# AnnaLew/pangenomix

Measured on AMD Instinct MI355X. Metric: proteins/sec clustered at 0.8 identity + pan/core iters/sec, 400-genome set, higher is better.
Workload: dtype i32

## Files before the change

pangenomix_amd/csrc/cluster.hip:

```cpp
#include <algorithm>
#include <chrono>
#include <cstdlib>
#include <cmath>
#include <type_traits>
#include <functional>
#include <condition_variable>
#include <mutex>
#include <thread>
#include <vector>

#include "cluster_layout.h"
#include "cluster_tables.h"
#include "pgx_internal.h"

namespace {

using namespace pgxc;

constexpr uint32_t kWindowMax = 65536;
constexpr int kDiscoveryRounds = 2;
constexpr uint32_t kBlockCap = 4096;
constexpr uint32_t kBlockCapMin = 64;

constexpr uint32_t kMaxLen = 1u << 22;
// ... 20 lines not shown
    uint32_t minc;
    int32_t best_sum, band_left, band_center, band_right;
    int32_t iden;
    uint32_t flags;
};

struct PairSel {
    const uint32_t *d_begin, *d_end;
    uint32_t cap;
    const uint32_t *list;
    uint32_t n_list;
    const uint8_t *only_a, *only_not_b;
    uint8_t *accepted_out;
    uint32_t b0;
    uint32_t skip_evaluated;
    uint32_t all_if_le;
};
__device__ __forceinline__ uint32_t sel_count(const PairSel &s) {
    if (s.list) return s.n_list;
    uint32_t e = *s.d_end;
    if (e > s.cap) e = s.cap;
    const uint32_t b = s.d_begin ? *s.d_begin : 0u;
    return e > b ? e - b : 0u;
}
__device__ __forceinline__ uint32_t sel_pair(const PairSel &s, uint32_t w) {
    return s.list ? s.list[w] : (s.d_begin ? *s.d_begin : 0u) + w;
}

struct DevSeqs {
    const uint8_t *res;
    const uint64_t *off;
    const uint32_t *len;
    const uint32_t *wcode;
    const uint16_t *wmult;
    const uint32_t *wcnt;
    const uint32_t *pk;
    const uint32_t *pk_off;
    uint32_t n_fwd;
    int32_t base;
    int32_t kd;
    int32_t nt;
    uint32_t mshift;
};
__device__ __forceinline__ uint32_t entry_rmask(const DevSeqs &S) { return (1u << S.mshift) - 1u; }
__device__ __forceinline__ uint32_t entry_fmax(const DevSeqs &S) { return 0xFFFFFFFFu >> S.mshift; }
__device__ __forceinline__ uint32_t real_of(const DevSeqs &S, uint32_t k) { return k >= S.n_fwd ? k - S.n_fwd : k; }

__constant__ int8_t kAa2Idx_dev[26] = {0, 2, 4, 3, 6, 13, 7, 8, 9, 20, 11, 10, 12,
                                       2, 20, 14, 5, 1, 15, 16, 20, 19, 17, 20, 18, 6};

__device__ __forceinline__ bool is_letter(uint8_t ch) {
    ch &= 0xDF;
    return ch >= 'A' && ch <= 'Z';
}

__global__ __launch_bounds__(256) void seq_len_kernel(const uint8_t *__restrict__ res,
                                                     const uint64_t *__restrict__ off, uint32_t n, uint64_t total,
                                                     uint32_t *__restrict__ len) {
    const uint32_t lane = threadIdx.x & 63u;
    const uint32_t i = blockIdx.x * 4u + (threadIdx.x >> 6);
    if (i >= n) return;
    const uint64_t b = off[i], e = off[i + 1];
    uint32_t c = 0;
    const uint64_t a0 = b & ~3ull;
    for (uint64_t a = a0 + 4ull * lane; a < e; a += 256) {
        uint32_t word = 0;
        if (a + 4 <= total) word = *reinterpret_cast<const uint32_t *>(res + a);
        else for (uint64_t p = a; p < total; ++p) word |= (uint32_t)res[p] << (8 * (p - a));
#pragma unroll
        for (int t = 0; t < 4; ++t) {
            const uint64_t p = a + t;
            c += (p >= b && p < e) && is_letter((uint8_t)(word >> (8 * t)));
        }
    }
    for (int d = 32; d > 0; d >>= 1) c += __shfl_xor(c, d);
    if (lane == 0) len[i] = c;
}

__global__ __launch_bounds__(256) void encode_gather_kernel(const uint8_t *__restrict__ in,
                                                           const uint64_t *__restrict__ in_off,
                                                           const uint32_t *__restrict__ order,
                                                           const uint64_t *__restrict__ out_off,
                                                           uint8_t *__restrict__ out, uint32_t n, int nt) {
    const uint32_t lane = threadIdx.x & 63u;
    const uint32_t k = blockIdx.x * 4u + (threadIdx.x >> 6);
    if (k >= n) return;
    const uint32_t src = order[k];
    const uint64_t b = in_off[src], e = in_off[src + 1];
    uint64_t w = out_off[k];
    for (uint64_t q0 = b; q0 < e; q0 += 256) {
        uint8_t chs[4];
#pragma unroll
        for (int j = 0; j < 4; ++j) { const uint64_t p = q0 + 64u * j + lane; chs[j] = p < e ? in[p] : (uint8_t)0; }
#pragma unroll
        for (int j = 0; j < 4; ++j) {
            const uint8_t ch = chs[j];
            const bool ok = is_letter(ch);
            const unsigned long long m = __ballot(ok);
            if (ok) {
                const uint8_t up = ch & 0xDF;
                const uint8_t idx = nt ? (uint8_t)(up == 'A' ? 0 : up == 'C' ? 1 : up == 'G' ? 2 : (up == 'T' || up == 'U') ? 3 : 4)
                                       : (uint8_t)kAa2Idx_dev[up - 'A'];
                out[w + __popcll(m & ((1ull << lane) - 1ull))] = idx;
            }
            w += __popcll(m);
        }
// ... 279 lines not shown
            if (cur == key) break;
            if (cur == kSentinel) {
                const uint32_t was = atomicCAS(&hk[slot], kSentinel, key);
                if (was == kSentinel || was == key) break;
            }
            slot = (slot + 1u) & (SLOTS - 1u);
        }
        atomicAdd(&hc[slot], 1u);
    }
    __syncthreads();
    constexpr uint32_t C = SLOTS / THREADS;
    const uint32_t beg = tid * C;
    uint32_t mine = 0;
    for (uint32_t i = beg; i < beg + C; ++i) mine += hk[i] != kSentinel;
    uint32_t total;
    uint32_t idx = block_excl_scan<THREADS>(mine, part, &total);
    if (tid == 0) wcnt[k] = total;
    for (uint32_t i = beg; i < beg + C; ++i)
        if (hk[i] != kSentinel) { wcode[o + idx] = hk[i]; wmult[o + idx] = (uint16_t)hc[i]; ++idx; }
}

template <uint32_t SLOTS>
__global__ __launch_bounds__(256) void words_wave_kernel(const uint8_t *__restrict__ res, const uint64_t *__restrict__ off,
                                                         const uint32_t *__restrict__ len, uint32_t k0, uint32_t k1,
                                                         int word_len, int base, int nt, uint32_t *__restrict__ wcode,
                                                         uint16_t *__restrict__ wmult, uint32_t *__restrict__ wcnt) {
    constexpr uint32_t kStage = (15 + SLOTS / 2 + 10 + 15) / 16 + 1;
    constexpr uint32_t kLoads = (kStage + 63) / 64;
    __shared__ uint4 table4[4][SLOTS / 4];
    __shared__ uint4 stage[4][kStage];
    const uint32_t lane = threadIdx.x & 63u, wv = threadIdx.x >> 6;
    const uint32_t k = k0 + blockIdx.x * 4u + wv;
    if (k >= k1) return;
    const uint64_t o = off[k];
    const uint32_t L = len[k], nw = L - (uint32_t)word_len + 1u;
    const uint8_t *s = res + o;
    const uint8_t *g = reinterpret_cast<const uint8_t *>(reinterpret_cast<uintptr_t>(s) & ~uintptr_t(15));
    const uint32_t sh = (uint32_t)(s - g), nv = (sh + L + 15u) / 16u;
    uint4 v[kLoads];
#pragma unroll
    for (uint32_t t = 0; t < kLoads; ++t) {
        v[t] = make_uint4(0, 0, 0, 0);
        if (lane + 64u * t < nv && lane + 64u * t < kStage) v[t] = reinterpret_cast<const uint4 *>(g)[lane + 64u * t];
    }
    uint32_t *tb = reinterpret_cast<uint32_t *>(table4[wv]);
#pragma unroll
    for (uint32_t t = 0; t < SLOTS / 4 / 64; ++t) table4[wv][lane + 64u * t] = make_uint4(kSentinel, kSentinel, kSentinel, kSentinel);
#pragma unroll
    for (uint32_t t = 0; t < kLoads; ++t) if (lane + 64u * t < kStage) stage[wv][lane + 64u * t] = v[t];
    __builtin_amdgcn_fence(__ATOMIC_RELEASE, "workgroup");
    __builtin_amdgcn_wave_barrier();
    __builtin_amdgcn_fence(__ATOMIC_ACQUIRE, "workgroup");
    const uint8_t *l = reinterpret_cast<const uint8_t *>(stage[wv]) + sh;
    for (uint32_t i = lane; i < nw; i += 64u) {
        uint32_t key = 0;
        bool bad = false;
        for (int t = 0; t < word_len; ++t) { const uint32_t r = l[i + t]; key = key * (uint32_t)base + r; bad |= r >= (uint32_t)base; }
        if (nt && bad) continue;
        uint32_t slot = (key * 0x9E3779B1u) >> 7 & (SLOTS - 1u);
        for (;;) {
            const uint32_t cur = tb[slot];
            if (cur != kSentinel && (cur >> 10) == key) { atomicAdd(&tb[slot], 1u); break; }
            if (cur == kSentinel) {
                const uint32_t was = atomicCAS(&tb[slot], kSentinel, key << 10 | 1u);
                if (was == kSentinel) break;
                if ((was >> 10) == key) { atomicAdd(&tb[slot], 1u); break; }
            }
            slot = (slot + 1u) & (SLOTS - 1u);
        }
    }
    __builtin_amdgcn_fence(__ATOMIC_RELEASE, "workgroup");
    __builtin_amdgcn_wave_barrier();
    __builtin_amdgcn_fence(__ATOMIC_ACQUIRE, "workgroup");
    uint32_t n_out = 0;
#pragma unroll 4
    for (uint32_t r = 0; r < SLOTS / 64u; ++r) {
        const uint32_t e = tb[r * 64u + lane];
        const bool occ = e != kSentinel;
        const unsigned long long m = __ballot(occ);
        if (occ) {
            const uint32_t at = n_out + (uint32_t)__popcll(m & ((1ull << lane) - 1ull));
            wcode[o + at] = e >> 10;
            wmult[o + at] = (uint16_t)(e & 1023u);
        }
        n_out += (uint32_t)__popcll(m);
    }
    if (lane == 0) wcnt[k] = n_out;
}

__global__ __launch_bounds__(1024) void words_huge_kernel(const uint8_t *__restrict__ res, const uint64_t *__restrict__ off,
                                                          const uint32_t *__restrict__ len, uint32_t k0, uint32_t k1,
                                                          int word_len, int base, int nt, uint32_t *__restrict__ scratch,
                                                          uint32_t slots, uint32_t *__restrict__ wcode,
                                                          uint16_t *__restrict__ wmult, uint32_t *__restrict__ wcnt,
                                                          uint32_t *__restrict__ err) {
    __shared__ uint32_t part[1024];
    const uint32_t k = k0 + blockIdx.x;
    if (k >= k1) return;
    const uint32_t tid = threadIdx.x;
    uint32_t *hk = scratch + (size_t)blockIdx.x * 2u * slots, *hc = hk + slots;
    const uint64_t o = off[k];
    const uint8_t *s = res + o;
    const uint32_t nw = len[k] - (uint32_t)word_len + 1u;
    for (uint32_t i = tid; i < slots; i += 1024) { hk[i] = kSentinel; hc[i] = 0u; }
    __threadfence();
    __syncthreads();
// ... 1618 lines not shown
        return 1e3 * std::chrono::duration<double>(std::chrono::steady_clock::now() - t).count();
    };
    const bool trace_phases = std::getenv("PGX_TRACE") != nullptr;
    double t_mark = 0.0;
    auto phase = [&](const char *what) {
        if (!trace_phases) return;
        const double now = ms_since(t_call0);
        fprintf(stderr, "[pgx] %-28s %8.2f ms\n", what, now - t_mark);
        t_mark = now;
    };
    pgx_cluster_stats S{};
    S.n_input = n_in;
    if (out_n_clusters) *out_n_clusters = 0;
    const unsigned nth = host_threads(n_in);
    parallel_for(n_in, nth, [&](unsigned, size_t b, size_t e) {
        for (size_t i = b; i < e; ++i) {
            out_cluster[i] = -1; out_member[i] = -1; out_identity[i] = 0.f;
            if (out_strand) out_strand[i] = 0;
        }
    });
    if (n_in == 0) { if (stats) *stats = S; return PGX_OK; }

    DevBuf d_res, d_off, d_len, d_wcode, d_wmult, d_wcnt, d_aa1, d_aas, d_aan, d_lines, d_pool[2], d_idx,
        d_newbits, d_touched, d_first, d_best_own, d_rcvis, d_counters, d_visits, d_pairsW, d_pairsK, d_blk_list,
        d_ulist, d_new_list, d_flags, d_gscratch, d_order, d_list, d_gather, d_pk, d_pkoff,
        d_counters2, d_best2, d_flags2, d_pairsW2, d_gscratch2,
        d_thr, d_hugewords, d_xsend, d_xrecv,
        d_hist, d_sortcnt, d_tilesum, d_runs;
    {
        DevBuf *all[] = {&d_res, &d_off, &d_len, &d_wcode, &d_wmult, &d_wcnt, &d_aa1, &d_aas, &d_aan, &d_lines,
                         &d_pool[0], &d_pool[1], &d_idx, &d_newbits, &d_touched, &d_first, &d_best_own, &d_rcvis,
                         &d_counters, &d_visits, &d_pairsW, &d_pairsK, &d_blk_list, &d_ulist, &d_new_list, &d_flags,
                         &d_gscratch, &d_order, &d_list, &d_gather, &d_pk, &d_pkoff,
                         &d_counters2, &d_best2, &d_flags2, &d_pairsW2, &d_gscratch2, &d_thr, &d_hugewords,
                         &d_xsend, &d_xrecv, &d_hist, &d_sortcnt, &d_tilesum, &d_runs};
        int sl = 1;
        for (DevBuf *b : all) { b->ctx = ctx; b->slot = sl++; }
    }
    uint32_t n_codes = 1;
    for (int t = 0; t < P->word_len; ++t) n_codes *= nt ? 4u : (uint32_t)kNAA1;
    static_assert(kSegs == 4, "eight codes per word of the round's map");
    const uint32_t bm_words = (n_codes / 8 + 2 + 3) & ~3u;
    const bool overlap = !nt && !std::getenv("PGX_NO_OVERLAP");
    DevBuf d_in_len;
    d_in_len.ctx = ctx; d_in_len.slot = 0;
    PGX_HIP(d_in_len.alloc((size_t)n_in * 4));
    constexpr uint32_t kHistWords = H_BINS + kDevSortMaxLen + 1;
    PGX_HIP(d_hist.alloc((size_t)kHistWords * 4));
    PGX_HIP(d_idx.alloc(16));
    PGX_HIP(d_newbits.alloc(2 * (size_t)bm_words * 4 + 16));
    PGX_HIP(d_counters.alloc(C_COUNT * 4));
    PGX_HIP(d_visits.alloc(8));
    if (overlap) PGX_HIP(d_counters2.alloc(C_COUNT * 4));
    {
        ClearArgs ca{};
        auto seg = [&](DevBuf &b, size_t words) { ca.p[ca.n] = b.as<uint32_t>(); ca.words[ca.n] = (uint32_t)words; ++ca.n; };
        seg(d_hist, kHistWords);
        seg(d_newbits, 2 * (size_t)bm_words);
        seg(d_counters, C_COUNT);
        seg(d_visits, 2);
        if (overlap) seg(d_counters2, C_COUNT);
        ca.one = d_idx.as<uint32_t>();
        clear_kernel<<<1024, 256, 0, st>>>(ca);
        LAUNCH_CHECK();
    }
    {
        ProfScope prof(ctx, "seq_len_kernel", st);
        seq_len_kernel<<<(n_in + 3) / 4, 256, 0, st>>>(d_residues, d_offsets, n_in, total_in, d_in_len.as<uint32_t>());
        len_hist_kernel<<<std::min(64u, (n_in + 1023u) / 1024u), 1024, 0, st>>>(d_in_len.as<uint32_t>(), n_in, P->min_length,
                                                                               d_hist.as<uint32_t>());
    }
    LAUNCH_CHECK();
    HostVec<uint32_t> h_hist(ctx, 6, kHistWords);
    PGX_REQUIRE(h_hist.ok(), "out of host memory");
    PGX_HIP(hipMemcpyAsync(h_hist.data(), d_hist.p, (size_t)(H_BINS + kHistLds) * 4, hipMemcpyDeviceToHost, st));
    PGX_HIP(hipStreamSynchronize(st));
    const bool dev_sort = h_hist[H_OVER] == 0 && !std::getenv("PGX_HOST_PROLOGUE");
    uint32_t max_len = h_hist[H_MAX];
    if (dev_sort && max_len >= kHistLds) {
        PGX_HIP(hipMemcpyAsync(h_hist.data() + H_BINS + kHistLds, d_hist.as<uint32_t>() + H_BINS + kHistLds,
                               (size_t)(max_len + 1 - kHistLds) * 4, hipMemcpyDeviceToHost, st));
        PGX_HIP(hipStreamSynchronize(st));
    }
    phase("  seq_len + histogram + copy");
    const uint32_t *len_hist = h_hist.data() + H_BINS;
    uint32_t n = 0;
    HostVec<uint32_t> order(ctx, 1, dev_sort ? 0 : n_in);
    std::vector<uint32_t> host_hist;
    if (dev_sort) {
        for (uint32_t L = 0; L <= max_len; ++L) n += len_hist[L];
    } else {
        HostVec<uint32_t> in_len(ctx, 0, n_in);
        PGX_REQUIRE(in_len.ok() && order.ok(), "out of host memory");
        PGX_HIP(hipMemcpyAsync(in_len.data(), d_in_len.p, (size_t)n_in * 4, hipMemcpyDeviceToHost, st));
        PGX_HIP(hipStreamSynchronize(st));
        max_len = 0;
        {
            std::vector<uint32_t> mx(nth, 0u);
            parallel_for(n_in, nth, [&](unsigned t, size_t b, size_t e) {
                uint32_t m = 0;
                for (size_t i = b; i < e; ++i) m = std::max(m, in_len[i]);
                mx[t] = m;
            });
            for (uint32_t m : mx) max_len = std::max(max_len, m);
        }
        if (max_len > kMaxLen) {
            pgx_set_error("pgx_cluster_greedy: sequence of %u residues exceeds the supported maximum %u", max_len, kMaxLen);
            return PGX_ERR_CAPACITY;
        }
        const size_t n_bkt = (size_t)max_len + 2;
        std::vector<uint32_t> bucket(n_bkt * nth, 0);
        parallel_for(n_in, nth, [&](unsigned t, size_t b, size_t e) {
            uint32_t *h = bucket.data() + n_bkt * t;
            for (size_t i = b; i < e; ++i)
                if ((int)in_len[i] > P->min_length) h[max_len - in_len[i]]++;
        });
        host_hist.assign((size_t)max_len + 1, 0u);
        for (size_t l = 0; l <= max_len; ++l)
            for (unsigned t = 0; t < nth; ++t) {
                const uint32_t c = bucket[n_bkt * t + l];
                bucket[n_bkt * t + l] = n; n += c; host_hist[max_len - l] += c;
            }
        parallel_for(n_in, nth, [&](unsigned t, size_t b, size_t e) {
            uint32_t *h = bucket.data() + n_bkt * t;
            for (size_t i = b; i < e; ++i)
                if ((int)in_len[i] > P->min_length) order[h[max_len - in_len[i]]++] = (uint32_t)i;
        });
        len_hist = host_hist.data();
    }
// ... 45 lines not shown
            PGX_REQUIRE(!(len_hist[L] && t_aas[L] < 1), "aas_cutoff too small: every sequence needs required_aas >= 1");
        S.sum_len_queries = run_off[n_runs];
    }
    S.n_clustered = n;

    const uint32_t window_cap = pgx_cluster_window_cap(P);
    PGX_REQUIRE(!exchanging || window_cap <= PGX_EXCHANGE_KEYS, "window larger than PGX_EXCHANGE_KEYS");
    uint32_t pair_cap = 4u << 20;
    uint32_t block_cap = std::min(nt ? 512u : kBlockCap, window_cap);
    const uint32_t pair_cap_k = nt ? 512u * 512u + 16u : (1u << 20);
    const double thr_frac = P->identity > 0.95 ? std::max(0.0, 1.0 - (1.0 - P->identity) * P->word_len) : P->aan_cutoff;
    static const double chunk_frac = std::getenv("PGX_CHUNK_FRAC") ? std::atof(std::getenv("PGX_CHUNK_FRAC")) : 0.8;
    double cur_frac = chunk_frac;
    uint64_t chunk_words = (uint64_t)(cur_frac * thr_frac * (double)n_codes);
    const bool chunking = chunk_words >= 16384;
    std::vector<uint32_t> flush_at(P->chunk_boundaries, P->chunk_boundaries + (P->chunk_boundaries ? P->n_chunk_boundaries : 0u));
    for (size_t i = 0; i < flush_at.size(); ++i)
        PGX_REQUIRE(flush_at[i] > 0 && flush_at[i] < n && (i == 0 || flush_at[i] > flush_at[i - 1]),
                    "chunk_boundaries must be strictly increasing positions in (0, number of clustered sequences)");
    auto form_window = [&](uint32_t b0, Chunks &C, uint32_t limit) -> uint32_t {
        C.n = 1; C.begin[0] = 0;
        uint64_t in_chunk = 0;
        uint32_t q = 0;
        for (; b0 + q < limit && q < window_cap; ++q) {
            const uint64_t w = h_len[b0 + q];
            if (chunking && in_chunk && in_chunk + w > chunk_words) {
                if (C.n == kMaxChunks) break;
                C.begin[C.n++] = q;
                in_chunk = 0;
            }
            in_chunk += w;
        }
        C.begin[C.n] = q;
        return q;
    };
    const bool need_gscratch = (uint64_t)max_len * 2 > kDiagLdsSmall;
    const uint32_t packed_len = nt ? kPackedLenNt : kPackedLenAa;
    const uint32_t gs_cells = (max_len + 64u) & ~63u;
    const uint32_t gs_stride = (max_len > packed_len ? 5u : 3u) * gs_cells;
    const uint32_t diag_grid = (uint32_t)std::max<uint64_t>(64, std::min<uint64_t>(8192, (4ull << 30) / ((uint64_t)gs_stride * 4)));
    const uint32_t align_grid = 1024;

    PGX_HIP(d_res.alloc(total + 16));
    PGX_HIP(d_off.alloc(((size_t)nv + 1) * 8));
    PGX_HIP(d_len.alloc((size_t)nv * 4));
    PGX_HIP(d_wcode.alloc((total + 16) * 4));
    PGX_HIP(d_wmult.alloc((total + 16) * 2));
    PGX_HIP(d_wcnt.alloc((size_t)nv * 4));
    PGX_HIP(d_pk.alloc(((size_t)total_pk + 16) * 4));
    PGX_HIP(d_pkoff.alloc(((size_t)nv + 1) * 4));
    PGX_HIP(d_aa1.alloc((size_t)n * 4));
    PGX_HIP(d_aas.alloc((size_t)n * 4));
    PGX_HIP(d_aan.alloc((size_t)n * 4));
    PGX_HIP(d_lines.alloc((size_t)n_codes * sizeof(IndexLine)));
    PGX_HIP(hipMemsetAsync(d_lines.p, 0, (size_t)n_codes * sizeof(IndexLine), st));
    PGX_HIP(d_best_own.alloc((size_t)window_cap * 8));
    PGX_HIP(d_rcvis.alloc((size_t)window_cap * 8));
    PGX_HIP(d_blk_list.alloc((size_t)kBlockCap * 4));
    PGX_HIP(d_ulist.alloc((size_t)window_cap * 4));
    PGX_HIP(d_new_list.alloc((size_t)window_cap * 4));
    PGX_HIP(d_flags.alloc(4 * (size_t)window_cap));
    PGX_HIP(d_list.alloc((size_t)pair_cap_k * 4));
    PGX_HIP(d_gather.alloc((size_t)pair_cap_k * sizeof(Pair)));
    PGX_HIP(d_pairsW.alloc((size_t)pair_cap * sizeof(Pair)));
    PGX_HIP(d_pairsK.alloc((size_t)pair_cap_k * sizeof(Pair)));
    if (need_gscratch) PGX_HIP(d_gscratch.alloc((size_t)diag_grid * gs_stride * 4));
    if (overlap) {
        if (!exchanging) PGX_HIP(d_best2.alloc((size_t)window_cap * 8));
        PGX_HIP(d_flags2.alloc(4 * (size_t)window_cap));
        PGX_HIP(d_pairsW2.alloc((size_t)pair_cap * sizeof(Pair)));
        if (need_gscratch) PGX_HIP(d_gscratch2.alloc((size_t)diag_grid * gs_stride * 4));
    }
    int pool_cur = 0;
    uint64_t pool_cap = 0;
    auto ensure_pool = [&](uint64_t entries, hipStream_t on) -> int {
        const uint64_t need = 8 * entries + 4096;
        if (need <= pool_cap) return PGX_OK;
        if (need > 0xFFFFFFF0ull) { pgx_set_error("pgx_cluster_greedy: word index too large for 32-bit pool offsets"); return PGX_ERR_CAPACITY; }
        const uint64_t want = std::min<uint64_t>(0xFFFFFFF0ull, need + need / 2);
        DevBuf &nb_ = d_pool[pool_cur ^ 1];
        PGX_HIP(nb_.alloc(want * 4));
        if (pool_cap) PGX_HIP(hipMemcpyAsync(nb_.p, d_pool[pool_cur].p, pool_cap * 4, hipMemcpyDeviceToDevice, on));
        pool_cur ^= 1;
        pool_cap = want;
        return PGX_OK;
    };
    PGX_HIP(d_order.alloc((size_t)n * 4));
    if (dev_sort) {
        uint32_t per = kSortShare;
        while ((uint64_t)((n_in + per - 1) / per) * n_runs > kSortCells) per *= 2;
        const uint32_t n_shares = (n_in + per - 1) / per, cells = n_shares * n_runs, tiles = (cells + kScanTile - 1) / kScanTile;
        PGX_HIP(d_sortcnt.alloc((size_t)cells * 4));
        PGX_HIP(d_tilesum.alloc((size_t)tiles * 4));
        uint32_t *const cnt = d_sortcnt.as<uint32_t>(), *const in_len = d_in_len.as<uint32_t>();
        ProfScope prof(ctx, "length_sort_kernels", st);
        ClearArgs ca{};
        ca.p[0] = cnt; ca.words[0] = cells; ca.n = 1;
        clear_kernel<<<std::min(2048u, (cells + 255u) / 256u), 256, 0, st>>>(ca);
        sort_count_kernel<<<(n_in + 255) / 256, 256, 0, st>>>(in_len, n_in, P->min_length, max_len, per, n_shares, cnt);
        tile_sum_kernel<<<tiles, 256, 0, st>>>(cnt, cells, d_tilesum.as<uint32_t>());
        tile_scan_kernel<<<tiles, 256, 0, st>>>(cnt, cells, d_tilesum.as<uint32_t>());
        sort_place_kernel<<<(n_shares + 3) / 4, 256, 0, st>>>(in_len, n_in, P->min_length, max_len, per, n_shares, cnt, n,
                                                              d_order.as<uint32_t>());
        LAUNCH_CHECK();
        PGX_HIP(hipMemcpyAsync(order.data(), d_order.p, (size_t)n * 4, hipMemcpyDeviceToHost, st));
    } else {
        PGX_HIP(hipMemcpyAsync(d_order.p, order.data(), (size_t)n * 4, hipMemcpyHostToDevice, st));
    }
    {
        const size_t runs_bytes = 2 * ((size_t)n_runs + 1) * 8;
        PGX_HIP(d_runs.alloc(runs_bytes));
        PGX_HIP(hipMemcpyAsync(d_runs.p, h_runs.data(), runs_bytes, hipMemcpyHostToDevice, st));
        const uint64_t *const dr_off = d_runs.as<uint64_t>();
        const uint32_t *const dr_pos = reinterpret_cast<const uint32_t *>(dr_off + n_runs + 1), *const dr_pk = dr_pos + n_runs + 1;
        layout_kernel<<<nv / 256 + 1, 256, 0, st>>>(dr_off, dr_pos, dr_pk, n_runs, max_len, n, nv, d_len.as<uint32_t>(),
                                                    d_off.as<uint64_t>(), d_pkoff.as<uint32_t>());
        LAUNCH_CHECK();
    }
    {
        ProfScope prof(ctx, "encode_gather_kernel", st);
        encode_gather_kernel<<<(n + 3) / 4, 256, 0, st>>>(d_residues, d_offsets, d_order.as<uint32_t>(),
                                                          d_off.as<uint64_t>(), d_res.as<uint8_t>(), n, nt ? 1 : 0);
        if (both)
            revcomp_kernel<<<(n + 3) / 4, 256, 0, st>>>(d_res.as<uint8_t>(), d_off.as<uint64_t>(),
                                                        d_len.as<uint32_t>(), n);
        pack5_kernel<<<(nv + 3) / 4, 256, 0, st>>>(d_res.as<uint8_t>(), d_off.as<uint64_t>(), d_len.as<uint32_t>(),
                                                   d_pkoff.as<uint32_t>(), nv, d_pk.as<uint32_t>());
    }
    LAUNCH_CHECK();
    {
        PGX_HIP(d_thr.alloc(3 * ((size_t)max_len + 1) * 4));
        PGX_HIP(hipMemcpyAsync(d_thr.p, h_thr.data(), 3 * ((size_t)max_len + 1) * 4, hipMemcpyHostToDevice, st));
        thresholds_kernel<<<(n + 255) / 256, 256, 0, st>>>(d_len.as<uint32_t>(), n, d_thr.as<int32_t>(), max_len + 1,
                                                          d_aa1.as<int32_t>(), d_aas.as<int32_t>(), d_aan.as<int32_t>());
        LAUNCH_CHECK();
    }
    phase("alloc + sort + layout + encode (enq)");
    {
        const int wl = P->word_len;
        auto first_with_words_le = [&](uint32_t cap) { return pgxc::first_with_words_le(run_pos, max_len, cap, wl); };
        const uint32_t k32 = first_with_words_le(32768), k8 = first_with_words_le(8192),
                       k2 = first_with_words_le(2048), k1k = first_with_words_le(1023), k5 = first_with_words_le(512);
        int rc;
        uint8_t *r8 = d_res.as<uint8_t>(); uint64_t *o64 = d_off.as<uint64_t>(); uint32_t *l32 = d_len.as<uint32_t>();
        uint32_t *wc = d_wcode.as<uint32_t>(); uint16_t *wm = d_wmult.as<uint16_t>(); uint32_t *wn = d_wcnt.as<uint32_t>();
        const int base = nt ? 4 : kNAA1;
        for (uint32_t half = 0; half < (both ? 2u : 1u); ++half) {
            const uint32_t o = half * n;
            if (k32) {
                uint32_t slots = 65536;
                while (slots < 2u * max_len) slots *= 2;
                const uint32_t per_launch = std::min(k32, std::max(1u, (uint32_t)((256ull << 20) / ((uint64_t)slots * 8))));
                PGX_HIP(d_hugewords.alloc((size_t)per_launch * slots * 8));
                ProfScope prof(ctx, "words_kernel", st);
                for (uint32_t a = 0; a < k32; a += per_launch)
                    words_huge_kernel<<<std::min(per_launch, k32 - a), 1024, 0, st>>>(r8, o64, l32, o + a, o + std::min(k32, a + per_launch), wl, base,
                                                                                       nt, d_hugewords.as<uint32_t>(), slots, wc, wm, wn,
                                                                                       d_counters.as<uint32_t>() + C_ERR);
                LAUNCH_CHECK();
            }
            if ((rc = launch_words<32768, 1024>(ctx, st, r8, o64, l32, o + k32, o + k8, wl, base, nt, wc, wm, wn))) return rc;
            if ((rc = launch_words<8192, 1024>(ctx, st, r8, o64, l32, o + k8, o + k2, wl, base, nt, wc, wm, wn))) return rc;
            if ((rc = launch_words_hash<2048, 256>(ctx, st, r8, o64, l32, o + k2, o + k1k, wl, base, nt, wc, wm, wn))) return rc;
            if (k5 > k1k) {
                ProfScope prof(ctx, "words_kernel", st);
                words_wave_kernel<2048><<<(k5 - k1k + 3) / 4, 256, 0, st>>>(r8, o64, l32, o + k1k, o + k5, wl, base, nt, wc, wm, wn);
                LAUNCH_CHECK();
            }
            if (n > k5) {
                ProfScope prof(ctx, "words_kernel", st);
                words_wave_kernel<1024><<<(n - k5 + 3) / 4, 256, 0, st>>>(r8, o64, l32, o + k5, o + n, wl, base, nt, wc, wm, wn);
                LAUNCH_CHECK();
            }
        }
    }
    DevSeqs DS{d_res.as<uint8_t>(), d_off.as<uint64_t>(), d_len.as<uint32_t>(),
               d_wcode.as<uint32_t>(), d_wmult.as<uint16_t>(), d_wcnt.as<uint32_t>(),
               d_pk.as<uint32_t>(), d_pkoff.as<uint32_t>(), n, nt ? 4 : kNAA1, nt ? 4 : 2, nt ? 1 : 0, mshift};
    HostVec<uint32_t> h_wcnt(ctx, 8, n);
    PGX_REQUIRE(h_wcnt.ok(), "out of host memory");
    PGX_HIP(hipMemcpyAsync(h_wcnt.data(), d_wcnt.p, (size_t)n * 4, hipMemcpyDeviceToHost, st));

    phase("word lists (enqueue)");
    fill_host_layout();
    phase("host lengths + offsets");
    uint64_t max_window_words = 0;
    uint32_t max_chunks = 1;
    {
        Chunks C;
        size_t nf = 0;
        for (uint32_t b0 = 0, nbw; b0 < n; b0 += nbw) {
            while (nf < flush_at.size() && flush_at[nf] <= b0) ++nf;
            nbw = form_window(b0, C, nf < flush_at.size() ? flush_at[nf] : n);
            max_window_words = std::max<uint64_t>(max_window_words, h_off[b0 + nbw] - h_off[b0]);
            max_chunks = std::max(max_chunks, C.n);
        }
        if (!flush_at.empty())
            max_window_words = std::max<uint64_t>(max_window_words, h_off[std::min(n, window_cap)]);
    }
    if (chunking && flush_at.empty())
        max_window_words = std::max<uint64_t>(max_window_words,
            std::min<uint64_t>(h_off[std::min(n, window_cap)], (uint64_t)kMaxChunks * std::max<uint64_t>(chunk_words, max_len)));
    PGX_REQUIRE(max_window_words < 0xFFFFFFF0ull, "window too large");
    PGX_HIP(d_touched.alloc((max_window_words + 16) * sizeof(Deferred)));
    if (chunking && n > window_cap / 2) max_chunks = kMaxChunks;
    uint32_t tag_stride = 1;
    while (tag_stride < max_chunks) tag_stride *= 2;
    PGX_HIP(d_first.alloc((size_t)tag_stride * n_codes * 4 + 16));
    std::vector<uint32_t> rep_seq;
    HostVec<int32_t> cluster_of(ctx, 9, n, -1);
    HostVec<int32_t> iden_of(ctx, 10, n, -1);
    PGX_REQUIRE(cluster_of.ok() && iden_of.ok(), "out of host memory");
    Pinned<Pair> hW, hK;
    Pinned<unsigned long long> h_best, h_rcvis;
    Pinned<uint32_t> h_cnt, h_blk, h_new, h_list, h_push;
    Pinned<Pair> h_gather;
// ... 19 lines not shown
        PGX_HIP(hipEventCreateWithFlags(&ev.post[i], hipEventDisableTiming));
    }
    const hipStream_t st_main = st;
    uint32_t *const dc_set[2] = {d_counters.as<uint32_t>(), d_counters2.as<uint32_t>()};
    unsigned long long *d_rcvis_p = d_rcvis.as<unsigned long long>();
    const uint32_t shard_count = P->shard_count > 0 ? (uint32_t)P->shard_count : 1u;
    if (native_exchange) {
        PGX_HIP(d_xsend.alloc((size_t)PGX_EXCHANGE_SLOTS * PGX_EXCHANGE_WORDS * 8));
        PGX_HIP(d_xrecv.alloc((size_t)PGX_EXCHANGE_SLOTS * shard_count * PGX_EXCHANGE_WORDS * 8));
    }
    unsigned long long *const x_send = native_exchange ? d_xsend.as<unsigned long long>() : static_cast<unsigned long long *>(P->exchange_send);
    const unsigned long long *const x_recv = native_exchange ? d_xrecv.as<unsigned long long>() : static_cast<const unsigned long long *>(P->exchange_recv);
    unsigned long long *d_best = exchanging ? x_send : d_best_own.as<unsigned long long>();
    const uint32_t shard_index = P->shard_count > 0 ? (uint32_t)P->shard_index : 0u;
    const bool count_replicated = shard_index == 0;
    int inject_rank = -1;
    uint64_t inject_at = 0, n_exchanges = 0;
    if (const char *e = std::getenv("PGX_INJECT_ERROR")) { unsigned long long at = 0; if (sscanf(e, "%d:%llu", &inject_rank, &at) == 2) inject_at = at; else inject_rank = -1; }
    uint64_t visits_rc = 0;
    unsigned long long *const d_best_set[2] = {d_best, exchanging ? d_best + PGX_EXCHANGE_WORDS : d_best2.as<unsigned long long>()};
    uint8_t *const d_flags_set[2] = {d_flags.as<uint8_t>(), d_flags2.as<uint8_t>()};
    std::vector<uint8_t> status(window_cap);
    HostVec<uint8_t> strand_of(ctx, 11, n, (uint8_t)0);
    PGX_REQUIRE(strand_of.ok(), "out of host memory");
    std::vector<unsigned long long> winner_key(window_cap);
    std::vector<uint32_t> new_reps, order_k, rank_of(window_cap), bucket_k(kBlockCap + 2), fill_k(kBlockCap + 2), flight;
    auto real = [&](uint32_t k) { return k >= n ? k - n : k; };
    auto pair_key = [&](const Pair &pp) {
        return ((unsigned long long)(pp.q >= n) << 63) | ((unsigned long long)pp.minc << 32) | pp.r;
    };
    uint64_t n_rounds = 0;

    uint64_t gpu_pairs = 0, gpu_aligned = 0, gpu_aligned_bytes = 0, filter_walk_words = 0;
    auto account = [&](const Pair *pp, uint32_t cnt) {
        for (uint32_t i = 0; i < cnt; ++i) {
            ++gpu_pairs;
            if ((pp[i].flags & (F_DIAG_PASS | F_BAND_OK)) != (F_DIAG_PASS | F_BAND_OK)) continue;
            ++gpu_aligned;
            gpu_aligned_bytes += h_len[pp[i].q] + h_len[pp[i].r];
        }
    };
    auto window_error = [&](uint32_t e, uint32_t at) {
        pgx_set_error("pgx_cluster_greedy: capacity failure in the window at %u%s:%s%s%s%s%s%s", at,
                      exchanging ? " (on this or another process)" : "",
                      e & E_TOUCHED ? " append scratch list full;" : "", e & E_POOL ? " overflow pool of the word index full;" : "",
                      e & E_TABLE ? " exact table of the filter overflowed;" : "",
                      e & E_BAND ? " alignment band wider than 64 diagonals;" : "", e & E_PAIRS ? " candidate pair buffer overflow;" : "",
                      e & E_WORDMULT ? " a word occurs more than 65535 times in one sequence;" : "");
    };
    const bool trace = std::getenv("PGX_TRACE") != nullptr;
    const uint32_t filter_grid = 4096u;
    uint32_t epoch_idx = 0;
    uint32_t epoch_tag = 0;
    PGX_HIP(hipMemsetAsync(d_first.p, 0, (size_t)tag_stride * n_codes * 4, st));
    phase("window set-up");
    const auto t_loop0 = std::chrono::steady_clock::now();
    double t_resolve = 0.0, t_close = 0.0;
    uint64_t n_blocks = 0;
    g_wait_s = 0.0;
    std::function<int()> deferred;
    std::vector<uint32_t> members;
    uint64_t pending_words = 0;
    Chunks chunks;
    Pinned<uint8_t> h_taken;
    h_taken.bind(ctx, 14);
    if (!flush_at.empty()) { PGX_HIP(h_taken.reserve(n)); std::fill(h_taken.p, h_taken.p + n, (uint8_t)0); }
    auto drain = [&]() -> int {
        if (deferred) { int rc = deferred(); deferred = nullptr; if (rc) return rc; }
        PGX_HIP(hipStreamSynchronize(st_main));
        PGX_HIP(hipStreamSynchronize(ctx->stream2));
        return PGX_OK;
    };
    size_t next_flush = 0;
    bool sweeping = false;
    uint32_t sweep_at = 0;
    for (uint32_t cursor = 0, nb = 0; cursor < n;) {
        if (!sweeping && next_flush < flush_at.size() && cursor == flush_at[next_flush]) {
            ++next_flush;
            sweeping = true; sweep_at = cursor;
            int rc = drain(); if (rc) return rc;
        }
        const bool sweep = sweeping;
        const uint32_t b0 = sweep ? sweep_at : cursor;
        nb = form_window(b0, chunks, sweep || next_flush >= flush_at.size() ? n : flush_at[next_flush]);
        const int set = overlap ? (int)(S.sweeps & 1u) : 0;
        const hipStream_t st = set ? ctx->stream2 : st_main;
        uint32_t *const dc = dc_set[set];
        unsigned long long *const d_best = d_best_set[set];
        uint8_t *const d_done = d_flags_set[set], *const d_inblk = d_done + window_cap;
        uint8_t *const d_hascand = d_done + 2 * (size_t)window_cap, *const d_accepted = d_done + 3 * (size_t)window_cap;
        Pinned<Pair> &hW_w = set ? hW2 : hW;
        Pinned<unsigned long long> &h_best_w = set ? h_best2 : h_best;
        Pinned<uint32_t> &h_ccnt_w = set ? h_ccnt2 : h_ccnt;
        uint32_t *const d_gs = (set ? d_gscratch2 : d_gscratch).as<uint32_t>();
        if (overlap && S.sweeps > 0)
            PGX_HIP(hipStreamWaitEvent(st, ev.strike[set ^ 1], 0));
        bool strike_recorded = false;
        const uint32_t ns = both ? 2 * nb : nb;
        const uint32_t n_reps = (uint32_t)rep_seq.size();
        const uint64_t window_words = h_off[b0 + nb] - h_off[b0];
        { int rc = ensure_pool(S.rep_words + pending_words + window_words, st); if (rc) return rc; }
        uint32_t *d_poolp = d_pool[pool_cur].as<uint32_t>();
        if (nt) {
            const uint64_t need = (uint64_t)ns * ((uint64_t)n_reps + nb) + 1024;
            if (need > (400ull << 20)) {
                pgx_set_error("pgx_cluster_greedy: %llu candidate pairs in one window exceed the supported maximum",
                              (unsigned long long)need);
// ... 530 lines not shown
```

Before: 16.40 million.

## Fuse encode, gather, pack and word counting for short sequences into one kernel

Adds prep_fused_kernel, which for short sequences (up to 1023 words) gathers raw residues, encodes letters through a packed constant lookup, writes the encoded residues and the 5-bit packed form, and builds the word table in one wave per sequence. The separate encode, pack and words kernels now only run on the long-sequence prefix. This removes global memory round trips and kernel launches. The change also moves the d_lines memset earlier so it overlaps the histogram copy, replaces a stream sync with a busy-wait event poll, and runs the d_first memset on a second stream. In exchange it adds complexity and uses more registers and LDS in the fused kernel.

```diff
diff --git a/pangenomix_amd/csrc/cluster.hip b/pangenomix_amd/csrc/cluster.hip
--- a/pangenomix_amd/csrc/cluster.hip
+++ b/pangenomix_amd/csrc/cluster.hip
@@ -96,6 +96,19 @@
 __device__ __forceinline__ bool is_letter(uint8_t ch) {
     ch &= 0xDF;
     return ch >= 'A' && ch <= 'Z';
+}
+
+constexpr uint64_t aa_pack12(int first) {
+    const int8_t tab[26] = {0, 2, 4, 3, 6, 13, 7, 8, 9, 20, 11, 10, 12, 2, 20, 14, 5, 1, 15, 16, 20, 19, 17, 20, 18, 6};
+    uint64_t v = 0;
+    for (int i = 0; i < 12 && first + i < 26; ++i) v |= (uint64_t)tab[first + i] << (5 * i);
+    return v;
+}
+__device__ __forceinline__ uint32_t aa_index(uint32_t i ) {
+    constexpr uint64_t t0 = aa_pack12(0), t1 = aa_pack12(12), t2 = aa_pack12(24);
+    const uint64_t t = i < 12u ? t0 : i < 24u ? t1 : t2;
+    const uint32_t j = i < 12u ? i : i < 24u ? i - 12u : i - 24u;
+    return (uint32_t)(t >> (5u * j)) & 31u;
 }
 
 __global__ __launch_bounds__(256) void seq_len_kernel(const uint8_t *__restrict__ res,
@@ -481,6 +494,137 @@
     __builtin_amdgcn_wave_barrier();
     __builtin_amdgcn_fence(__ATOMIC_ACQUIRE, "workgroup");
     const uint8_t *l = reinterpret_cast<const uint8_t *>(stage[wv]) + sh;
+    for (uint32_t i = lane; i < nw; i += 64u) {
+        uint32_t key = 0;
+        bool bad = false;
+        for (int t = 0; t < word_len; ++t) { const uint32_t r = l[i + t]; key = key * (uint32_t)base + r; bad |= r >= (uint32_t)base; }
+        if (nt && bad) continue;
+        uint32_t slot = (key * 0x9E3779B1u) >> 7 & (SLOTS - 1u);
+        for (;;) {
+            const uint32_t cur = tb[slot];
+            if (cur != kSentinel && (cur >> 10) == key) { atomicAdd(&tb[slot], 1u); break; }
+            if (cur == kSentinel) {
+                const uint32_t was = atomicCAS(&tb[slot], kSentinel, key << 10 | 1u);
+                if (was == kSentinel) break;
+                if ((was >> 10) == key) { atomicAdd(&tb[slot], 1u); break; }
+            }
+            slot = (slot + 1u) & (SLOTS - 1u);
+        }
+    }
+    __builtin_amdgcn_fence(__ATOMIC_RELEASE, "workgroup");
+    __builtin_amdgcn_wave_barrier();
+    __builtin_amdgcn_fence(__ATOMIC_ACQUIRE, "workgroup");
+    uint32_t n_out = 0;
+#pragma unroll 4
+    for (uint32_t r = 0; r < SLOTS / 64u; ++r) {
+        const uint32_t e = tb[r * 64u + lane];
+        const bool occ = e != kSentinel;
+        const unsigned long long m = __ballot(occ);
+        if (occ) {
+            const uint32_t at = n_out + (uint32_t)__popcll(m & ((1ull << lane) - 1ull));
+            wcode[o + at] = e >> 10;
+            wmult[o + at] = (uint16_t)(e & 1023u);
+        }
+        n_out += (uint32_t)__popcll(m);
+    }
+    if (lane == 0) wcnt[k] = n_out;
+}
+
+template <uint32_t SLOTS>
+__global__ __launch_bounds__(256) __attribute__((amdgpu_waves_per_eu(SLOTS == 1024 ? 8 : 4, 8))) void prep_fused_kernel(const uint8_t *__restrict__ in, const uint64_t *__restrict__ in_off,
+                                                         uint64_t in_total, const uint32_t *__restrict__ order,
+                                                         const uint64_t *__restrict__ off, const uint32_t *__restrict__ len,
+                                                         const uint32_t *__restrict__ pk_off, uint32_t k0, uint32_t k1,
+                                                         int word_len, int base, int nt, uint8_t *__restrict__ res,
+                                                         uint32_t *__restrict__ pk, uint32_t *__restrict__ wcode,
+                                                         uint16_t *__restrict__ wmult, uint32_t *__restrict__ wcnt) {
+    constexpr uint32_t kStage = (15 + SLOTS / 2 + 10 + 15) / 16 + 1;
+    __shared__ uint4 table4[4][SLOTS / 4];
+    __shared__ uint4 stage[4][kStage];
+    const uint32_t lane = threadIdx.x & 63u, wv = threadIdx.x >> 6;
+    const uint32_t k = k0 + blockIdx.x * 4u + wv;
+    if (k >= k1) return;
+    const uint64_t o = off[k];
+    const uint32_t sh = (uint32_t)(reinterpret_cast<uintptr_t>(res + o) & 15u);
+    const uint32_t L = min(len[k], kStage * 16u - 15u), nw = L - (uint32_t)word_len + 1u;
+    const uint32_t pko = pk_off[k];
+    uint32_t *tb = reinterpret_cast<uint32_t *>(table4[wv]);
+#pragma unroll
+    for (uint32_t t = 0; t < SLOTS / 4 / 64; ++t) table4[wv][lane + 64u * t] = make_uint4(kSentinel, kSentinel, kSentinel, kSentinel);
+    uint8_t *l = reinterpret_cast<uint8_t *>(stage[wv]) + sh;
+    {
+        const uint32_t src = order[k];
+        const uintptr_t p0 = reinterpret_cast<uintptr_t>(in), pb = p0 + in_off[src], pe = p0 + in_off[src + 1], pt = p0 + in_total;
+        uint32_t w = 0;
+        for (uintptr_t a0 = pb & ~uintptr_t(15); a0 < pe && w < L; a0 += 1024u) {
+            const uintptr_t a = a0 + 16u * lane;
+            uint32_t x[4] = {0u, 0u, 0u, 0u};
+            if (a < pe) {
+                if (a >= p0 && a + 16u <= pt) {
+                    const uint4 v = *reinterpret_cast<const uint4 *>(a);
+                    x[0] = v.x; x[1] = v.y; x[2] = v.z; x[3] = v.w;
+                } else {
+#pragma unroll
+                    for (uint32_t j = 0; j < 4; ++j) {
+                        const uintptr_t aj = a + 4u * j;
+                        if (aj >= p0 && aj + 4u <= pt) x[j] = *reinterpret_cast<const uint32_t *>(aj);
+                        else for (uintptr_t p = aj < p0 ? p0 : aj; p < pt && p < aj + 4u; ++p)
+                            x[j] |= (uint32_t)*reinterpret_cast<const uint8_t *>(p) << (8u * (uint32_t)(p - aj));
+                    }
+                }
+            }
+            const uint32_t lo = a < pb ? (uint32_t)(pb - a) : 0u, hi = a >= pe ? 0u : pe - a > 16u ? 16u : (uint32_t)(pe - a);
+            const uint32_t in_span = ((1u << hi) - 1u) & ~((1u << lo) - 1u);
+            uint32_t mine = 0, before = 0, all = 0;
+#pragma unroll
+            for (uint32_t t = 0; t < 16; ++t) {
+                const bool ok = (in_span >> t & 1u) && is_letter((uint8_t)(x[t >> 2] >> (8u * (t & 3u))));
+                const unsigned long long m = __ballot(ok);
+                mine |= (ok ? 1u : 0u) << t;
+                before += (uint32_t)__popcll(m & ((1ull << lane) - 1ull));
+                all += (uint32_t)__popcll(m);
+            }
+            uint32_t at = w + before;
+#pragma unroll 1
+            for (uint32_t j = 0; j < 4; ++j) {
+#pragma unroll 1
+                for (uint32_t t = 0; t < 4; ++t) {
+                    if (mine & 1u) {
+                        const uint8_t up = (uint8_t)x[0] & 0xDF;
+                        const uint8_t idx = nt ? (uint8_t)(up == 'A' ? 0 : up == 'C' ? 1 : up == 'G' ? 2 : (up == 'T' || up == 'U') ? 3 : 4)
+                                               : (uint8_t)aa_index((uint32_t)up - 'A');
+                        if (at < L) l[at] = idx;
+                        ++at;
+                    }
+                    mine >>= 1; x[0] >>= 8;
+                }
+                x[0] = x[1]; x[1] = x[2]; x[2] = x[3];
+            }
+            w += all;
+        }
+    }
+    __builtin_amdgcn_fence(__ATOMIC_RELEASE, "workgroup");
+    __builtin_amdgcn_wave_barrier();
+    __builtin_amdgcn_fence(__ATOMIC_ACQUIRE, "workgroup");
+    {
+        uint8_t *g = res + o - sh;
+        const uint32_t nv = (sh + L + 15u) / 16u;
+        for (uint32_t p = lane; p < nv; p += 64u) {
+            if (16u * p >= sh && 16u * p + 16u <= sh + L) reinterpret_cast<uint4 *>(g)[p] = stage[wv][p];
+            else for (uint32_t j = 16u * p < sh ? sh : 16u * p; j < 16u * p + 16u && j < sh + L; ++j) g[j] = l[j - sh];
+        }
+    }
+    {
+        uint32_t *dst = pk + pko;
+        const uint32_t np = (L + 5u) / 6u;
+        for (uint32_t w = lane; w < np; w += 64u) {
+            uint32_t x = 0;
+#pragma unroll
+            for (uint32_t t = 0; t < 6; ++t)
+                if (6u * w + t < L) x |= (uint32_t)l[6u * w + t] << (5u * t);
+            dst[w] = x;
+        }
+    }
     for (uint32_t i = lane; i < nw; i += 64u) {
         uint32_t key = 0;
         bool bad = false;
@@ -2205,6 +2349,13 @@
     PGX_HIP(d_counters.alloc(C_COUNT * 4));
     PGX_HIP(d_visits.alloc(8));
     if (overlap) PGX_HIP(d_counters2.alloc(C_COUNT * 4));
+    PGX_HIP(d_lines.alloc((size_t)n_codes * sizeof(IndexLine)));
+    struct OneEvent {
+        hipEvent_t e = nullptr;
+        ~OneEvent() { if (e) (void)hipEventDestroy(e); }
+    } ev_hist, ev_first;
+    PGX_HIP(hipEventCreateWithFlags(&ev_hist.e, hipEventDisableTiming));
+    PGX_HIP(hipEventCreateWithFlags(&ev_first.e, hipEventDisableTiming));
     {
         ClearArgs ca{};
         auto seg = [&](DevBuf &b, size_t words) { ca.p[ca.n] = b.as<uint32_t>(); ca.words[ca.n] = (uint32_t)words; ++ca.n; };
@@ -2227,7 +2378,14 @@
     HostVec<uint32_t> h_hist(ctx, 6, kHistWords);
     PGX_REQUIRE(h_hist.ok(), "out of host memory");
     PGX_HIP(hipMemcpyAsync(h_hist.data(), d_hist.p, (size_t)(H_BINS + kHistLds) * 4, hipMemcpyDeviceToHost, st));
-    PGX_HIP(hipStreamSynchronize(st));
+    PGX_HIP(hipEventRecord(ev_hist.e, st));
+    PGX_HIP(hipMemsetAsync(d_lines.p, 0, (size_t)n_codes * sizeof(IndexLine), st));
+    {
+        hipError_t e;
+        while ((e = hipEventQuery(ev_hist.e)) == hipErrorNotReady) {
+        }
+        PGX_HIP(e);
+    }
     const bool dev_sort = h_hist[H_OVER] == 0 && !std::getenv("PGX_HOST_PROLOGUE");
     uint32_t max_len = h_hist[H_MAX];
     if (dev_sort && max_len >= kHistLds) {
@@ -2379,8 +2537,6 @@
     PGX_HIP(d_aa1.alloc((size_t)n * 4));
     PGX_HIP(d_aas.alloc((size_t)n * 4));
     PGX_HIP(d_aan.alloc((size_t)n * 4));
-    PGX_HIP(d_lines.alloc((size_t)n_codes * sizeof(IndexLine)));
-    PGX_HIP(hipMemsetAsync(d_lines.p, 0, (size_t)n_codes * sizeof(IndexLine), st));
     PGX_HIP(d_best_own.alloc((size_t)window_cap * 8));
     PGX_HIP(d_rcvis.alloc((size_t)window_cap * 8));
     PGX_HIP(d_blk_list.alloc((size_t)kBlockCap * 4));
@@ -2444,15 +2600,22 @@
                                                     d_off.as<uint64_t>(), d_pkoff.as<uint32_t>());
         LAUNCH_CHECK();
     }
-    {
+    const int wl = P->word_len;
+    auto first_with_words_le = [&](uint32_t cap) { return pgxc::first_with_words_le(run_pos, max_len, cap, wl); };
+    const uint32_t k32 = first_with_words_le(32768), k8 = first_with_words_le(8192),
+                   k2 = first_with_words_le(2048), k1k = first_with_words_le(1023), k5 = first_with_words_le(512);
+    const bool fused = !both && !std::getenv("PGX_SPLIT_PREP");
+    const uint32_t n_split = fused ? k1k : n;
+    if (n_split) {
         ProfScope prof(ctx, "encode_gather_kernel", st);
-        encode_gather_kernel<<<(n + 3) / 4, 256, 0, st>>>(d_residues, d_offsets, d_order.as<uint32_t>(),
-                                                          d_off.as<uint64_t>(), d_res.as<uint8_t>(), n, nt ? 1 : 0);
+        encode_gather_kernel<<<(n_split + 3) / 4, 256, 0, st>>>(d_residues, d_offsets, d_order.as<uint32_t>(),
+                                                                d_off.as<uint64_t>(), d_res.as<uint8_t>(), n_split, nt ? 1 : 0);
         if (both)
             revcomp_kernel<<<(n + 3) / 4, 256, 0, st>>>(d_res.as<uint8_t>(), d_off.as<uint64_t>(),
                                                         d_len.as<uint32_t>(), n);
-        pack5_kernel<<<(nv + 3) / 4, 256, 0, st>>>(d_res.as<uint8_t>(), d_off.as<uint64_t>(), d_len.as<uint32_t>(),
-                                                   d_pkoff.as<uint32_t>(), nv, d_pk.as<uint32_t>());
+        const uint32_t n_pack = both ? nv : n_split;
+        pack5_kernel<<<(n_pack + 3) / 4, 256, 0, st>>>(d_res.as<uint8_t>(), d_off.as<uint64_t>(), d_len.as<uint32_t>(),
+                                                       d_pkoff.as<uint32_t>(), n_pack, d_pk.as<uint32_t>());
     }
     LAUNCH_CHECK();
     {
@@ -2464,10 +2627,6 @@
     }
     phase("alloc + sort + layout + encode (enq)");
     {
-        const int wl = P->word_len;
-        auto first_with_words_le = [&](uint32_t cap) { return pgxc::first_with_words_le(run_pos, max_len, cap, wl); };
-        const uint32_t k32 = first_with_words_le(32768), k8 = first_with_words_le(8192),
-                       k2 = first_with_words_le(2048), k1k = first_with_words_le(1023), k5 = first_with_words_le(512);
         int rc;
         uint8_t *r8 = d_res.as<uint8_t>(); uint64_t *o64 = d_off.as<uint64_t>(); uint32_t *l32 = d_len.as<uint32_t>();
         uint32_t *wc = d_wcode.as<uint32_t>(); uint16_t *wm = d_wmult.as<uint16_t>(); uint32_t *wn = d_wcnt.as<uint32_t>();
@@ -2489,6 +2648,19 @@
             if ((rc = launch_words<32768, 1024>(ctx, st, r8, o64, l32, o + k32, o + k8, wl, base, nt, wc, wm, wn))) return rc;
             if ((rc = launch_words<8192, 1024>(ctx, st, r8, o64, l32, o + k8, o + k2, wl, base, nt, wc, wm, wn))) return rc;
             if ((rc = launch_words_hash<2048, 256>(ctx, st, r8, o64, l32, o + k2, o + k1k, wl, base, nt, wc, wm, wn))) return rc;
+            if (fused) {
+                ProfScope prof(ctx, "prep_fused_kernel", st);
+                if (k5 > k1k)
+                    prep_fused_kernel<2048><<<(k5 - k1k + 3) / 4, 256, 0, st>>>(d_residues, d_offsets, total_in, d_order.as<uint32_t>(), o64,
+                                                                                l32, d_pkoff.as<uint32_t>(), k1k, k5, wl, base, nt, r8,
+                                                                                d_pk.as<uint32_t>(), wc, wm, wn);
+                if (n > k5)
+                    prep_fused_kernel<1024><<<(n - k5 + 3) / 4, 256, 0, st>>>(d_residues, d_offsets, total_in, d_order.as<uint32_t>(), o64,
+                                                                              l32, d_pkoff.as<uint32_t>(), k5, n, wl, base, nt, r8,
+                                                                              d_pk.as<uint32_t>(), wc, wm, wn);
+                LAUNCH_CHECK();
+                continue;
+            }
             if (k5 > k1k) {
                 ProfScope prof(ctx, "words_kernel", st);
                 words_wave_kernel<2048><<<(k5 - k1k + 3) / 4, 256, 0, st>>>(r8, o64, l32, o + k1k, o + k5, wl, base, nt, wc, wm, wn);
@@ -2614,7 +2786,9 @@
     const uint32_t filter_grid = 4096u;
     uint32_t epoch_idx = 0;
     uint32_t epoch_tag = 0;
-    PGX_HIP(hipMemsetAsync(d_first.p, 0, (size_t)tag_stride * n_codes * 4, st));
+    PGX_HIP(hipMemsetAsync(d_first.p, 0, (size_t)tag_stride * n_codes * 4, ctx->stream2));
+    PGX_HIP(hipEventRecord(ev_first.e, ctx->stream2));
+    PGX_HIP(hipStreamWaitEvent(st, ev_first.e, 0));
     phase("window set-up");
     const auto t_loop0 = std::chrono::steady_clock::now();
     double t_resolve = 0.0, t_close = 0.0;
```

New measurement: 16.49 million, median of 4. No clear change (+0.6%).
